# Codes4Fun/moshi.cpp

Measured on AMD Instinct MI355X. Metric: audio frames/sec (12.5 Hz target) moshika-7B q4_k decode, higher is better.
Workload: dtype q4_K weights x q8_K activations (int8 dot, f32 accumulate); bf16 KV; f32 elsewhere; 1 GPU; moshi-sts --bench loop: mimi encode + Temporal step + 8 Depth steps + mimi decode, moshika q4_k, 1 audio stream per GPU, greedy, ctx capacity 3000; context_fill_start=0, parallelism=1 GPU, device= (gfx950:sramecc+:xnack-)

## Files before the change

moshi.cpp_amd/csrc/hip_backend.hip:

```cpp
#include "hip_common.h"
#include "ggml-cpu.h"

#include <string.h>

#include <algorithm>
#include <functional>
#include <deque>
#include <map>
#include <memory>
#include <set>
#include <string>
#include <unordered_map>
#include <vector>

#define UPLOAD_SLOTS       8
#define UPLOAD_BLOB_BYTES  (64 * 1024)
#define UPLOAD_MAX_DESCS   1024
#define READBACK_PINNED_BYTES (64 * 1024)
#define AGET_SLOTS 64
#define AGET_SLOT_BYTES 256
#define UPLOAD_SMALL_MAX   16384

struct plan_t;

// ... 2516 lines not shown
            const ggml_tensor * n = g->nodes[i];
            const bool layout = is_layout_op(n->op);
            if (!layout || it != pl.at_pos.end())
                fprintf(stderr, "plan %4d %-18s [%5lld %5lld %4lld %2lld] %s%s%s\n", i, ggml_op_name(n->op), (long long) n->ne[0], (long long) n->ne[1], (long long) n->ne[2],
                        (long long) n->ne[3], pl.an.skip[(size_t) i] ? "fused" : (layout ? "-" : "GENERIC"), it != pl.at_pos.end() ? " <emit group>" : "", n->view_src ? " (alias)" : "");
        }
        if (!pl.an.skip[(size_t) i]) {
            if (g->nodes[i]->op == GGML_OP_SOFT_MAX || g->nodes[i]->op == GGML_OP_SET_ROWS) pl.p->n_generic_attn_nodes++;
            emit_generic(pl.em, g->nodes[i]);
        }
        if (it != pl.at_pos.end()) for (auto & f : it->second) pl.p->steps.push_back(f);
    }
}

static void hoist_rope_tables(planner & pl) {
    plan_t * p = pl.p;
    for (size_t i = 1; i + 1 < p->steps.size(); i++) {
        pstep & h = p->steps[i];
        const pstep & m = p->steps[i - 1];
        if (!h.hoist_dst || !m.is_mv || m.mv.special || m.mv.wtype != GGML_TYPE_F32 || m.mv.ncols != 2 || !p->steps[i + 1].is_mv) continue;
        auto clash = [&](const float * q, int64_t n_floats) { return q && (const char *) q < h.hoist_dst + h.hoist_bytes && h.hoist_dst < (const char *) (q + n_floats); };
        const mv_args & a = m.mv;
        if (clash(a.x, a.x_cs * (a.ncols - 1) + a.K) || clash(a.y, a.y_cs * (a.ncols - 1) + a.M) || clash(a.x_out, a.K * a.ncols) || clash(a.residual, a.r_cs * (a.ncols - 1) + a.M) ||
            clash(a.alpha, a.K) || clash(a.beta, a.K)) continue;
        std::swap(p->steps[i - 1], p->steps[i]);
    }
}

static bool chains_wanted(const planner & pl) {
    return pl.fuse && pl.keep && !(pl.c->flags & 16) && ((pl.c->flags & 32) || k_chain_default_on()) && spin_kernels_possible(pl.c);
// ... 377 lines not shown
```

moshi.cpp_amd/csrc/hip_chain.hip:

```cpp
#include "hip_common.h"
#include "hip_device.h"
#include "hip_mv_device.h"
#include "hip_attn_body.h"

#include <stdlib.h>
#include <string.h>
#include <type_traits>
#include <map>
#include <vector>

#define CH_NCW       8
#define CH_THREADS   (CH_NCW * 64)
#define CH_PMAX_OF(G) ((G) >= 256 ? 2 : (G) >= 128 ? 3 : 6)
#define CH_XF_MAX    4096
#define CH_PART_MAX  2048
#define CH_RES_MAX   256
#define CH_ATTW      1408
#define CH_SPIN_MAX  (1u << 24)
#define CH_MAX_PHASES 4095

typedef unsigned long long u64;

#if defined(CH_LOG)
__device__ u64 g_ch_log[2][512][16];
// ... 1135 lines not shown
        if (!mimi_is_mv(op, D, D, MV_PLAIN) || op.x != at.out || op.x_cs != D || op.residual != xin || op.r_cs != xin_cs || op.out_act) { if (verbose && d.L == 0) fprintf(stderr, "mimi_match: rule %d fails at layer 0\n", 8); break; }
        if (!mimi_is_mv(l1, D, F, MV_LAYERNORM) || !l1.alpha || l1.x != op.y || l1.x_cs != D || l1.residual || l1.out_scale || l1.out_act != 1) { if (verbose && d.L == 0) fprintf(stderr, "mimi_match: rule %d fails at layer 0\n", 9); break; }
        if (!mimi_is_mv(l2, F, D, MV_PLAIN) || l2.x != l1.y || l2.x_cs != F || l2.residual != op.y || l2.r_cs != D || l2.out_act) { if (verbose && d.L == 0) fprintf(stderr, "mimi_match: rule %d fails at layer 0\n", 10); break; }
        if (d.L == 0 && d.x_cs < D) { if (verbose && d.L == 0) fprintf(stderr, "mimi_match: rule %d fails at layer 0\n", 11); break; }
        d.mv.push_back({ ip.w, ip.alpha, ip.beta, nullptr, ip.y, ip.x_out, ip.eps, { 0, 0, 0 } });
        d.mv.push_back({ op.w, nullptr, nullptr, op.out_scale, op.y, nullptr, 0.f, { 0, 0, 0 } });
        d.mv.push_back({ l1.w, l1.alpha, l1.beta, nullptr, l1.y, l1.x_out, l1.eps, { 0, 0, 0 } });
        d.mv.push_back({ l2.w, nullptr, nullptr, l2.out_scale, l2.y, nullptr, 0.f, { 0, 0, 0 } });
        d.at.push_back({ at.kcache, at.vcache, at.rot, at.mask, at.index, at.out });
        d.weight_bytes += ip.M * ip.row_bytes + op.M * op.row_bytes + l1.M * l1.row_bytes + l2.M * l2.row_bytes;
        xprev = l2.y; xprev_cs = D;
        d.L++;
        i += 5;
    }
    if (d.L < 2) return 0;
    d.len = i;
    return i;
}
static size_t mimi_attn_smem(const attn_args & at) { return ATTN_RING256_SMEM + (size_t) at.C * 4 + (size_t) at.T * at.D * 4 * 3 + (size_t) CH_NCW * 64 * 8 * 8 + 16 + (size_t) at.T * at.C * 4 + 64; }
static size_t mimi_smem_bytes(const mimi_desc & d) {
    return (size_t) (2 * MIMI_F + 8) * 4 + 16 * 8 + sizeof(chain_ctl) + ((mimi_attn_smem(d.at0) + 15) & ~(size_t) 15) + d.mv.size() * sizeof(mimi_mv) + d.at.size() * sizeof(mimi_at);
}
static size_t mimi_tables_bytes(const mimi_desc & d) { return GGML_PAD(d.mv.size() * sizeof(mimi_mv) + d.at.size() * sizeof(mimi_at), 256); }
static bool mimi_resident(const mimi_desc & d, int usable_cus) {
    const size_t smem = mimi_smem_bytes(d);
    if (smem > 159 * 1024) return false;
    static bool granted = false;
    if (!granted) { HIP_CHECK(hipFuncSetAttribute((const void *) mimi_tr_kernel, hipFuncAttributeMaxDynamicSharedMemorySize, 159 * 1024)); granted = true; }
    static const int force = chain_env("MI355X_CHAIN_GRID_FORCE", 0);
    int per_cu = 0;
    return force || (hipOccupancyMaxActiveBlocksPerMultiprocessor(&per_cu, (const void *) mimi_tr_kernel, CH_THREADS, smem) == hipSuccess && (long long) per_cu * usable_cus >= 256);
}

struct smp_strip { std::vector<mv_args> mv; std::vector<const sample_args *> smp; std::vector<int> end_of; bool any = false; };
static unsigned g_sampled_ticket;
static void sampled_strip(const mv_args * mv, int n, smp_strip & o) {
    for (int i = 0; i < n; i++) {
        const mv_args & a = mv[i];
        if (!a.special) { o.mv.push_back(a); o.smp.push_back(nullptr); o.end_of.push_back(i + 1); continue; }
        if (a.special != 3 || o.mv.empty() || o.smp.back() || !a.smp) break;
        mv_args & hd = o.mv.back();
        const sample_args & sa = *a.smp;
        if (hd.ticket || hd.argmax_out[0] || hd.argmax_out[1] || sa.logits != hd.y || sa.n != hd.M || sa.n != 2048 || sa.k < 1 || sa.k > 256 || !sa.noise || !sa.out) break;
        hd.ticket = &g_sampled_ticket; hd.argmax_out[0] = sa.out; hd.argmax_out[1] = sa.out2;
        o.smp.back() = a.smp; o.end_of.back() = i + 1; o.any = true;
    }
// ... 214 lines not shown
            char * state = base + mimi_tables_bytes(d);
            std::vector<char> tab(mimi_tables_bytes(d), 0);
            memcpy(tab.data(), d.mv.data(), d.mv.size() * sizeof(mimi_mv));
            memcpy(tab.data() + d.mv.size() * sizeof(mimi_mv), d.at.data(), d.at.size() * sizeof(mimi_at));
            c->nest_tables.swap(tab);
            HIP_CHECK(hipMemcpyAsync(base, c->nest_tables.data(), c->nest_tables.size(), hipMemcpyHostToDevice, s));
            HIP_CHECK(hipMemsetAsync(state, 0, chain_state_bytes(256), s));
            mimi_params & N = c->MM;
            memset(&N, 0, sizeof(N));
            N.P.phases = nullptr; N.P.n_phases = d.len;
            N.P.launch_seq = (unsigned *) state; N.P.gbuf = (u64 *) (state + 256); N.P.cand = N.P.gbuf + 2 * CH_XF_MAX; N.P.err = err; N.P.delay = 0;
            N.tables = (const u32x4 *) base;
            N.n_layers = d.L; N.x_in = d.x_in; N.x_cs = d.x_cs;
            N.at = d.at0; N.at.q = N.at.k = N.at.v = nullptr;
            N.first_partial = d.first_partial ? 1 : 0;
            if (d.first_partial) { N.q0 = d.at_first.q; N.k0 = d.at_first.k; N.v0 = d.at_first.v; }
            N.q_off = d.q_off; N.k_off = d.k_off; N.v_off = d.v_off;
            N.attn_smem = mimi_attn_smem(d.at0);
            N.ring256 = chain_env("MI355X_ATTN_RING256", 1) && d.at0.C > 64 && d.at0.C <= 256 ? 1 : 0;
            {
                static const int dflt[2] = { 30, 200 };
                N.delay[0] = dflt[0]; N.delay[1] = dflt[1];
                if (const char * e = getenv("MI355X_MIMI_DELAY")) { int v[2]; const int got = sscanf(e, "%d,%d", &v[0], &v[1]); for (int i = 0; i < got && i < 2; i++) N.delay[i] = v[i] < 0 ? 0 : v[i] > 600 ? 600 : v[i]; }
            }
            c->P = N.P;
            c->smem = mimi_smem_bytes(d);
            c->mimi = true; c->n80_weight_bytes = d.weight_bytes; c->n80_len = d.len;
            if (chain_env("MI355X_CHAIN_VERBOSE", 0)) fprintf(stderr, "chain engine: Mimi transformer program, %d layers, ring of %d, %zu bytes of LDS, %d plan steps\n", d.L, d.at0.C, c->smem, d.len);
            return c;
        }
    }
    {
        n80_desc d;
        if (n > 0 && (mv[0].special == 2 || (!mv[0].special && mv[0].wtype == GGML_TYPE_Q8_0)) && c->grid == 256 && nest80_match(mv, n, d) == n) {
            char * base = (char *) ws;
            char * state = base + nest80_tables_bytes(d);
            char * din = state + chain_state_bytes(256);
            std::vector<char> tab(nest80_tables_bytes(d), 0);
            char * t = tab.data();
            memcpy(t, d.ph.data(), d.ph.size() * sizeof(nest_ph)); t += d.ph.size() * sizeof(nest_ph);
            memcpy(t, d.at.data(), d.at.size() * sizeof(n80_at)); t += d.at.size() * sizeof(n80_at);
            memcpy(t, d.st.data(), d.st.size() * sizeof(n80_st)); t += d.st.size() * sizeof(n80_st);
            memcpy(t, d.dsets.data(), d.dsets.size() * 8);
// ... 72 lines not shown
    for (size_t i = 0; i < c->phases.size(); i++) {
        chain_phase & ph = c->phases[i];
        if (ph.attn >= 0) ph.at = c->attns[(size_t) ai++];
        ph.n_in = i > 0 ? c->phases[i - 1].n_pub : 0;
        ph.kind = chain_shape_kind(ph, c->grid);
        if (ph.emb_chain) { ph.prev_out[0] = c->phases[i - 1].argmax_out[0]; ph.prev_out[1] = c->phases[i - 1].argmax_out[1]; }
    }
}
void k_chain_free(chain_plan * c) { delete c; }
int k_chain_length(const chain_plan * c) { return c->P.n_phases; }
int64_t k_chain_weight_bytes(const chain_plan * c) { if (c->nest80 || c->mimi) return c->n80_weight_bytes; int64_t b = 0; for (auto & ph : c->phases) b += (int64_t) ph.M * ph.row_bytes; return b; }

bool k_chain_is_step_program(const chain_plan * c) { return c->nest || c->nest80 || c->mimi; }

void k_chain_launch(hipStream_t s, const chain_plan * c) {
    if (c->mimi) { mimi_tr_kernel<<<256, CH_THREADS, c->smem, s>>>(c->MM); return; }
    if (c->nest80) { depth_nest80_kernel<2048, 2048><<<256, CH_THREADS, c->smem, s>>>(c->N80); return; }
    if (c->nest) {
        if (c->NP.head_argmax == 2) depth_nest_kernel<256, true><<<c->grid, CH_THREADS, c->nest_smem, s>>>(c->NP);
        else depth_nest_kernel<256><<<c->grid, CH_THREADS, c->nest_smem, s>>>(c->NP);
        return;
    }
    if (c->grid == 256) matvec_chain_kernel<256><<<c->grid, CH_THREADS, c->smem, s>>>(c->P);
    else if (c->grid == 128) matvec_chain_kernel<128><<<c->grid, CH_THREADS, c->smem, s>>>(c->P);
    else matvec_chain_kernel<64><<<c->grid, CH_THREADS, c->smem, s>>>(c->P);
}

#define VQC_CPW 4
#define VQC_LEVELS_MAX 32
struct vqc_level { const char * emb; long long emb_row_bytes; const float * add_c; const float * num; float * resid_out; float * idx_f; int32_t * idx_i; long long pad; };
static_assert(sizeof(vqc_level) == 64, "level records are read by 16-byte lanes");
// ... 133 lines not shown
```

moshi.cpp_amd/csrc/hip_chain_mimi.h:

```cpp
#pragma once

struct mimi_mv { const char * w; const float * alpha; const float * beta; const float * out_scale; float * y; float * x_out; float eps; int pad[3]; };
struct mimi_at { char * kcache; char * vcache; const float * rot; const float * mask; const int32_t * index; float * out; };
static_assert(sizeof(mimi_mv) == 64 && sizeof(mimi_at) == 48, "tables are copied to LDS by 16-byte lanes");

struct mimi_params {
    chain_params P;
    const u32x4 * tables;
    int n_layers;
    const float * x_in; int64_t x_cs;
    attn_args at;
    int q_off, k_off, v_off;
    size_t attn_smem;
    int ring256;
    int first_partial;
    const float * q0, * k0, * v0;
    int delay[2];
};
#define MIMI_D 512
#define MIMI_F 2048

__global__ void __launch_bounds__(CH_THREADS) mimi_tr_kernel(mimi_params N) {
    constexpr int G = 256, D = MIMI_D, F = MIMI_F, T = 2;
    extern __shared__ __attribute__((aligned(16))) char smem[];
    const int tid = threadIdx.x, lane = tid & 63;
    const int wave = __builtin_amdgcn_readfirstlane(tid >> 6);
    const int wg = blockIdx.x;
    const int L = N.n_layers;

    float * xs = (float *) smem;
    float * xres = xs + T * F;
    double * stat = (double *) (xres + 8);
    chain_ctl * ctl = (chain_ctl *) (stat + 16);
    char * at_smem = (char *) (ctl + 1);
    const mimi_mv * t_mv = (const mimi_mv *) (at_smem + ((N.attn_smem + 15) & ~(size_t) 15));
    const mimi_at * t_at = (const mimi_at *) (t_mv + 4 * L);

    const chain_params & P = N.P;
    auto nbar = [&]() { lds_barrier(); };
    if (tid == 0) { ctl->failed = 0; ctl->token = 0; }
    {
        const int n16 = (4 * L * (int) sizeof(mimi_mv) + L * (int) sizeof(mimi_at)) / 16;
        const GLOBAL_AS u32x4 * src = (const GLOBAL_AS u32x4 *) N.tables;
        for (int i = tid; i < n16; i += CH_THREADS) ((u32x4 *) t_mv)[i] = src[i];
    }
    const unsigned launch = *gp(P.launch_seq);
    const unsigned tag_base = launch << 12;
    __syncthreads();

    auto ld_mv = [&](int q) {
        mimi_mv r;
        unsigned w[16];
        const unsigned * s = (const unsigned *) (t_mv + q);
#pragma unroll
        for (int i = 0; i < 16; i++) w[i] = (unsigned) __builtin_amdgcn_readfirstlane((int) s[i]);
        __builtin_memcpy(&r, w, sizeof(r));
        return r;
    };
    auto ld_w = [&](int q) -> const char * {
        const unsigned * s = (const unsigned *) (t_mv + q);
        unsigned w[2] = { (unsigned) __builtin_amdgcn_readfirstlane((int) s[0]), (unsigned) __builtin_amdgcn_readfirstlane((int) s[1]) };
        const char * r;
        __builtin_memcpy(&r, w, 8);
        return r;
    };
    auto ld_at = [&](int q) {
        mimi_at r;
        unsigned w[12];
        const unsigned * s = (const unsigned *) (t_at + q);
#pragma unroll
        for (int i = 0; i < 12; i++) w[i] = (unsigned) __builtin_amdgcn_readfirstlane((int) s[i]);
        __builtin_memcpy(&r, w, sizeof(r));
        return r;
    };
    auto give_up = [&]() { if (lane == 0) { lds_store(&ctl->failed, 1u); *gp(P.err) = 2u; } };

    f32x4 wr[8];
    auto request = [&](auto kvc, const char * w, int rows) {
        constexpr int KV = decltype(kvc)::value;
        const int row = wg * rows + (wave < rows ? wave : rows - 1);
        const GLOBAL_AS char * src = gp(w) + (long long) row * (KV * 256 * 4);
#pragma unroll
        for (int it = 0; it < KV; it++) wr[it] = __builtin_nontemporal_load((const GLOBAL_AS f32x4 *) (src + ((long long) it * 256 + lane * 4) * 4));
    };
    if (N.first_partial) request(std::integral_constant<int, 2>(), ld_w(1), 2); else request(std::integral_constant<int, 2>(), ld_w(0), 6);

    const int col = wave >> 2, t256 = (wave & 3) * 64 + lane;
    auto poll_cols = [&](auto kvc, int p, float xr[], int delay) {
        constexpr int KV = decltype(kvc)::value;
        for (int i = 0; i < delay; i++) __builtin_amdgcn_s_sleep(1);
        const unsigned tag_in = tag_base | (unsigned) p;
        const u64 * gin = P.gbuf + (size_t) ((p - 1) & 1) * CH_XF_MAX + (size_t) col * (KV * 256) + t256;
        u64 g[KV];
        unsigned spins = 0;
        for (;;) {
#pragma unroll
            for (int j = 0; j < KV; j++) g[j] = __hip_atomic_load(gin + 256 * j, __ATOMIC_RELAXED, __HIP_MEMORY_SCOPE_AGENT);
            bool ok = true;
#pragma unroll
            for (int j = 0; j < KV; j++) ok = ok && (unsigned) (g[j] >> 32) == tag_in;
            if (__all(ok)) break;
            if (++spins > CH_SPIN_MAX || lds_load(&ctl->failed)) { give_up(); break; }
            __builtin_amdgcn_s_sleep(1);
        }
        settle_vmcnt();
#pragma unroll
        for (int j = 0; j < KV; j++) xr[j] = __uint_as_float((unsigned) g[j]);
    };
    auto col_sum = [&](double v, int slot) -> double {
        v = wave_allsum_f64(v);
        if (lane == 0) stat[slot * 8 + wave] = v;
        nbar();
        const double * s4 = stat + slot * 8 + col * 4;
        return s4[0] + s4[1] + s4[2] + s4[3];
    };
    auto layer_norm = [&](float xr[2], const mimi_mv & mv) {
        const float al[2] = { gp(mv.alpha)[t256], gp(mv.alpha)[t256 + 256] };
        float be[2] = { 0.f, 0.f };
        if (mv.beta) { be[0] = gp(mv.beta)[t256]; be[1] = gp(mv.beta)[t256 + 256]; }
        double acc = 0;
#pragma unroll
        for (int j = 0; j < 2; j++) acc += (double) xr[j];
        acc = col_sum(acc, 0);
        const float mean = (float) (acc / (double) D);
        acc = 0;
#pragma unroll
        for (int j = 0; j < 2; j++) { const float v = xr[j] - mean; acc += (double) (v * v); }
        acc = col_sum(acc, 1);
        const float scale = 1.0f / sqrtf((float) (acc / (double) D) + mv.eps);
#pragma unroll
        for (int j = 0; j < 2; j++) { float v = ((xr[j] - mean) * scale) * al[j]; if (mv.beta) v = v + be[j]; xr[j] = v; }
    };
    auto row_dot = [&](auto kvc, float out[2]) {
        constexpr int KV = decltype(kvc)::value, K = KV * 256;
        double acc[2] = { 0, 0 };
#pragma unroll
        for (int it = 0; it < KV; it++) {
            const int k = it * 256 + lane * 4;
#pragma unroll
            for (int c = 0; c < 2; c++) {
                const float4 xv = *(const float4 *) (xs + c * K + k);
                acc[c] += (double) (wr[it][0] * xv.x);
                acc[c] += (double) (wr[it][1] * xv.y);
                acc[c] += (double) (wr[it][2] * xv.z);
                acc[c] += (double) (wr[it][3] * xv.w);
            }
// ... 2 lines not shown
        for (int c = 0; c < 2; c++) out[c] = (float) wave_allsum_f64(acc[c]);
    };
    auto publish = [&](int p, int M, int row, const float v[2]) {
        const unsigned tag_out = tag_base | (unsigned) (p + 1);
        u64 * go = P.gbuf + (size_t) (p & 1) * CH_XF_MAX;
#pragma unroll
        for (int c = 0; c < 2; c++) st_granule(go + (size_t) c * M + row, tag_out, __float_as_uint(v[c]));
    };
    [[maybe_unused]] constexpr int grid = G;
    const int owner_idx = wg >> 4;
    const bool owner = (wg & 15) == (owner_idx & 7);

    int p = 0;
#pragma unroll 1
    for (int l = 0; l < L; l++) {
        if (l == 0 && N.first_partial) {
            if (wave < 2) {
#pragma unroll
                for (int c = 0; c < 2; c++) if (lane == c) xres[c * 2 + wave] = gp(N.x_in)[(int64_t) c * N.x_cs + wg * 2 + wave];
            }
            p = __builtin_amdgcn_readfirstlane(p + 1);
        } else {
            CH_STAMP(10);
            const mimi_mv mv = ld_mv(4 * l);
            float xr[2];
            if (l == 0) { xr[0] = gp(N.x_in)[(int64_t) col * N.x_cs + t256]; xr[1] = gp(N.x_in)[(int64_t) col * N.x_cs + t256 + 256]; }
            else poll_cols(std::integral_constant<int, 2>(), p, xr, N.delay[0]);
            if (l == 0 && wave < 2) {
#pragma unroll
                for (int c = 0; c < 2; c++) if (lane == c) xres[c * 2 + wave] = gp(N.x_in)[(int64_t) c * N.x_cs + wg * 2 + wave];
            }
            CH_STAMP(2);
            layer_norm(xr, mv);
            xs[col * D + t256] = xr[0]; xs[col * D + t256 + 256] = xr[1];
            if (mv.x_out && wg == 0) { gp(mv.x_out)[(int64_t) col * D + t256] = xr[0]; gp(mv.x_out)[(int64_t) col * D + t256 + 256] = xr[1]; }
            nbar();
            CH_STAMP(5);
            if (wave < 6) {
                float o[2];
                row_dot(std::integral_constant<int, 2>(), o);
                const int row = wg * 6 + wave;
                if (lane == 0) { publish(p, 3 * D, row, o); gp(mv.y)[row] = o[0]; gp(mv.y)[3 * D + row] = o[1]; }
            }
            request(std::integral_constant<int, 2>(), ld_w(4 * l + 1), 2);
            CH_STAMP(8);
            p = __builtin_amdgcn_readfirstlane(p + 1);
        }
        {
            CH_STAMP(10);
            if (owner) {
                const mimi_at ta = ld_at(l);
                attn_args at = N.at;
                at.kcache = ta.kcache; at.vcache = ta.vcache; at.rot = ta.rot; at.mask = ta.mask; at.index = ta.index; at.out = ta.out;
                at.q = nullptr; at.k = nullptr; at.v = nullptr;
                at.row_split = 1; at.n_groups = 0; at.write_only = 0;
                const attn_split_ws w0 = { nullptr, nullptr, nullptr, 1, P.err, 0, 1 << 30, 1 << 30 };
                const attn_gqkv gq = { P.gbuf + (size_t) ((p - 1) & 1) * CH_XF_MAX, (int64_t) N.q_off, (int64_t) N.k_off, (int64_t) N.v_off, P.err };
                attn_gout go = { P.gbuf + (size_t) (p & 1) * CH_XF_MAX, tag_base | (unsigned) (p + 1), (int64_t) D };
#if defined(CH_LOG)
                go.log = wg == 0 && p < 512 ? &g_ch_log[0][p][0] : nullptr;
#endif
                __syncthreads();
                if (l == 0 && N.first_partial) {
                    at.q = N.q0; at.k = N.k0; at.v = N.v0;
                    if (N.ring256) attn_ring256_body<AT_GOUT>(at, at_smem, owner_idx >> 1, owner_idx & 1, 0u, attn_gqkv(), go);
                    else attn_decode_body<false, CH_NCW, AT_GOUT>(at, w0, at_smem, owner_idx >> 1, 0, owner_idx & 1, 0u, attn_gqkv(), go);
                } else if (N.ring256) attn_ring256_body<AT_GQKV | AT_GOUT>(at, at_smem, owner_idx >> 1, owner_idx & 1, tag_base | (unsigned) p, gq, go);
                else attn_decode_body<false, CH_NCW, AT_GQKV | AT_GOUT>(at, w0, at_smem, owner_idx >> 1, 0, owner_idx & 1, tag_base | (unsigned) p, gq, go);
                __syncthreads();
                CH_STAMP(8);
            }
            p = __builtin_amdgcn_readfirstlane(p + 1);
        }
        {
            CH_STAMP(10);
            const mimi_mv mv = ld_mv(4 * l + 1);
            float osc = 1.f;
            if (mv.out_scale && wave < 2) osc = gp(mv.out_scale)[wg * 2 + wave];
            float xr[2];
            poll_cols(std::integral_constant<int, 2>(), p, xr, owner ? 0 : N.delay[1]);
            CH_STAMP(2);
            xs[col * D + t256] = xr[0]; xs[col * D + t256 + 256] = xr[1];
            nbar();
            CH_STAMP(5);
            if (wave < 2) {
                float o[2];
                row_dot(std::integral_constant<int, 2>(), o);
                const int row = wg * 2 + wave;
                if (lane == 0) {
#pragma unroll
                    for (int c = 0; c < 2; c++) { float s = o[c]; if (mv.out_scale) s = s * osc; s = xres[c * 2 + wave] + s; o[c] = s; xres[c * 2 + wave] = s; }
                    publish(p, D, row, o); gp(mv.y)[row] = o[0]; gp(mv.y)[D + row] = o[1];
                }
            }
            request(std::integral_constant<int, 2>(), ld_w(4 * l + 2), 8);
            CH_STAMP(8);
            p = __builtin_amdgcn_readfirstlane(p + 1);
        }
        {
            CH_STAMP(10);
            const mimi_mv mv = ld_mv(4 * l + 2);
            float xr[2];
            poll_cols(std::integral_constant<int, 2>(), p, xr, N.delay[0]);
            CH_STAMP(2);
            layer_norm(xr, mv);
            xs[col * D + t256] = xr[0]; xs[col * D + t256 + 256] = xr[1];
            if (mv.x_out && wg == 0) { gp(mv.x_out)[(int64_t) col * D + t256] = xr[0]; gp(mv.x_out)[(int64_t) col * D + t256 + 256] = xr[1]; }
            nbar();
            {
                float o[2];
                row_dot(std::integral_constant<int, 2>(), o);
                const int row = wg * 8 + wave;
                if (lane == 0) { o[0] = gelu_table(o[0]); o[1] = gelu_table(o[1]); publish(p, F, row, o); gp(mv.y)[row] = o[0]; gp(mv.y)[F + row] = o[1]; }
            }
            request(std::integral_constant<int, 8>(), ld_w(4 * l + 3), 2);
            CH_STAMP(8);
            p = __builtin_amdgcn_readfirstlane(p + 1);
        }
        {
            CH_STAMP(10);
            const mimi_mv mv = ld_mv(4 * l + 3);
            float osc = 1.f;
            if (mv.out_scale && wave < 2) osc = gp(mv.out_scale)[wg * 2 + wave];
            float xr[8];
            poll_cols(std::integral_constant<int, 8>(), p, xr, N.delay[0]);
            CH_STAMP(2);
#pragma unroll
            for (int j = 0; j < 8; j++) xs[col * F + t256 + 256 * j] = xr[j];
            nbar();
            if (wave < 2) {
                float o[2];
                row_dot(std::integral_constant<int, 8>(), o);
                const int row = wg * 2 + wave;
                if (lane == 0) {
#pragma unroll
                    for (int c = 0; c < 2; c++) { float s = o[c]; if (mv.out_scale) s = s * osc; s = xres[c * 2 + wave] + s; o[c] = s; xres[c * 2 + wave] = s; }
                    if (l + 1 < L) publish(p, D, row, o);
                    gp(mv.y)[row] = o[0]; gp(mv.y)[D + row] = o[1];
                }
            }
            if (l + 1 < L) request(std::integral_constant<int, 2>(), ld_w(4 * l + 4), 6);
            nbar();
            CH_STAMP(8);
            p = __builtin_amdgcn_readfirstlane(p + 1);
        }
    }
    if (wg == 0 && tid == 0) *gp(P.launch_seq) = launch + 1u;
}
```

moshi.cpp_amd/csrc/moshi_hot.cpp:

```cpp
#include "moshi_hot.h"
#include "delay_ring.h"
#include "gguf.h"
#include "ggml-cpu.h"

#include <dlfcn.h>
#include <math.h>
#include <stdlib.h>
#include <string.h>

#include <deque>
#include <functional>
#include <map>
#include <set>
#include <string>
#include <vector>

typedef struct ggml_tensor * T;

namespace {

struct Rng {
    uint64_t s;
    explicit Rng(uint64_t seed) : s(seed) {}
    uint64_t next() { uint64_t z = (s += 0x9E3779B97F4A7C15ull); z = (z ^ (z >> 30)) * 0xBF58476D1CE4E5B9ull; z = (z ^ (z >> 27)) * 0x94D049BB133111EBull; return z ^ (z >> 31); }
// ... 734 lines not shown
    int (*rccl_all_reduce)(const void *, void *, size_t, int, int, void *, void *) = nullptr;
    moshi_hot_allreduce_t tp_allreduce = nullptr; void * tp_allreduce_user = nullptr;
    int64_t tp_reductions = 0;
    Transformer temporal_tp; T tp_x = nullptr, tp_msg = nullptr; std::vector<Builder *> g_tp;
    bool tp_frame = false; T tp_in = nullptr; Builder * g_tp_pre = nullptr, * g_tp_import = nullptr, * g_tp_post = nullptr; int64_t tp_frames = 0;
    DelayProtocol proto; DelayRing ring;
    struct Column { DelayRing ring; int64_t pos = 0; bool open = false, held = false; };
    int n_streams = 1; ModelKind kind = ModelKind::single; std::vector<Column> cols;
    struct Sampling { moshi_hot_sampling s; bool seeded = false; };
    std::vector<Sampling> sampling; bool any_seeded = false, sampling_dirty = true;
    T inv_temp_text = nullptr, inv_temp = nullptr;

    Rvq rvq_first, rvq_rest;
    ConvTr upsample; Conv downsample;
    Transformer dec_tr, enc_tr;
    std::vector<Conv> dec_convs; std::vector<ConvTr> dec_convtrs; std::vector<ResBlock> dec_res;
    std::vector<Conv> enc_convs; std::vector<ResBlock> enc_res;
    Builder * g_dec = nullptr; T dec_codes = nullptr, dec_frame = nullptr; int dec_T = 0;
    Builder * g_enc = nullptr; T enc_frame = nullptr, enc_codes = nullptr; int enc_T = 0;
    T enc_latent[2] = { nullptr, nullptr };

    std::vector<int32_t> tokens_tmp;
    std::vector<int32_t> pipe_codes, pipe_tokens; bool pipe_have_codes = false, pipe_have_tokens = false; float pipe_vad = 0.f;
    bool temporal_staged = false;
    std::function<void()> after_temporal_launch;
    int32_t last_text = 0; std::vector<int32_t> last_audio;
    bool timing = false; double phase_us[4] = { 0, 0, 0, 0 }; int64_t phase_n[4] = { 0, 0, 0, 0 };
};

#define STREAMS_REFUSE(ret) do { if (m->n_streams > 1) return ret; } while (0)

namespace {

T state(moshi_hot_model * m, enum ggml_type type, int64_t n0, int64_t n1 = 1, int64_t n2 = 1) {
    T t = ggml_new_tensor_3d(m->st_ctx, type, n0, n1, n2);
    return t;
}
T state4(moshi_hot_model * m, enum ggml_type type, int64_t n0, int64_t n1, int64_t n2, int64_t n3) {
    T t = ggml_new_tensor_4d(m->st_ctx, type, n0, n1, n2, n3);
    return t;
}

bool owns_step(const moshi_hot_config & c, int k) { return c.dep_shard_world <= 1 || k % c.dep_shard_world == c.dep_shard_rank; }

void make_transformer(moshi_hot_model * m, Transformer & tr, const std::string & name, int dim, int heads, int n_layers, int ffn_hidden,
                      int capacity, int max_period, int n_weight_sets, bool mimi_style, enum ggml_type wtype, int cross_len = 0, bool norms_only = false) {
    Weights & W = *m->W;
    tr.dim = dim; tr.heads = heads; tr.capacity = capacity; tr.max_period = max_period;
    tr.layers.resize((size_t) n_layers);
    const float s_in = 1.f / sqrtf((float) dim);
    const float upd = m->cfg.update_scale > 0.f ? m->cfg.update_scale : 1.f;
    auto qgen = [](float sd) { return [sd](T t, Rng & r, std::vector<uint8_t> & o) { gen_quant(t, r, o, sd); }; };
    auto ones = [](T t, Rng &, std::vector<uint8_t> & o) { gen_const(t, 1.f, o); };
    auto zeros = [](T t, Rng &, std::vector<uint8_t> & o) { gen_const(t, 0.f, o); };
    for (int l = 0; l < n_layers; l++) {
        Layer & L = tr.layers[(size_t) l];
        const std::string p = name + ".layers." + std::to_string(l) + ".";
        if (mimi_style) {
// ... 218 lines not shown
    m->g_dec = new Builder(m->be_codec, 256);
    Builder & g = *m->g_dec;
    T codes = ggml_new_tensor_2d(g, GGML_TYPE_I32, 1, c.mimi_n_q);
    m->dec_codes = codes;
    const int64_t B = codes->ne[2], K = codes->ne[1], Tn = codes->ne[0];
    T first = ggml_view_3d(g, codes, Tn, 1, B, codes->nb[1], codes->nb[2], 0);
    T emb = rvq_decode(g, m->rvq_first, first);
    if (K > 1) {
        T rest = ggml_view_3d(g, codes, Tn, K - 1, B, codes->nb[1], codes->nb[2], codes->nb[1] * 1);
        emb = ggml_add(g, emb, rvq_decode(g, m->rvq_rest, rest));
    }
    emb = streaming_conv_transpose(g, m->upsample, emb);
    m->dec_T = (int) emb->ne[0];
    T x = ggml_cont(g, ggml_transpose(g, emb));
    x = transformer_graph_build(g, m->dec_tr, x);
    x = ggml_transpose(g, x);
    x = streaming_conv(g, m->dec_convs[0], x);
    x = ggml_elu(g, x);
    for (int i = 0; i < 4; i++) {
        x = streaming_conv_transpose(g, m->dec_convtrs[(size_t) i], x);
        x = resnet_block(g, m->dec_res[(size_t) i], x);
        x = ggml_elu(g, x);
    }
    x = streaming_conv(g, m->dec_convs[1], x);
    m->dec_frame = x;
    g.expand(x);
    g.alloc();
}

void build_encode_graph(moshi_hot_model * m) {
// ... 1 lines not shown
    m->g_enc = new Builder(m->be_codec, 256);
    Builder & g = *m->g_enc;
    T x = ggml_new_tensor_1d(g, GGML_TYPE_F32, 1920);
    m->enc_frame = x;
    x = streaming_conv(g, m->enc_convs[0], x);
    for (int i = 0; i < 4; i++) {
        x = resnet_block(g, m->enc_res[(size_t) i], x);
        x = ggml_elu(g, x);
        x = streaming_conv(g, m->enc_convs[(size_t) (1 + i)], x);
    }
    x = ggml_elu(g, x);
    x = streaming_conv(g, m->enc_convs[5], x);
    m->enc_T = (int) x->ne[0];
    x = ggml_cont(g, ggml_transpose(g, x));
    x = transformer_graph_build(g, m->enc_tr, x);
    x = ggml_transpose(g, x);
    x = streaming_conv(g, m->downsample, x);
    T codes = rvq_encode(g, m->rvq_first, x, &m->enc_latent[0]);
    if (c.mimi_n_q > 1) codes = ggml_concat(g, codes, rvq_encode(g, m->rvq_rest, x, &m->enc_latent[1]), 1);
    codes = ggml_cast(g, codes, GGML_TYPE_I32);
    m->enc_codes = codes;
    g.expand(codes);
    g.alloc();
}

}

extern "C" void moshi_hot_config_moshika(struct moshi_hot_config * c) {
    memset(c, 0, sizeof(*c));
    c->dim = 4096; c->num_heads = 32; c->num_layers = 32; c->ffn_hidden = 11264; c->context = 3000; c->max_period = 10000;
// ... 265 lines not shown
        p.delays.assign(c.delays, c.delays + p.cols());
        for (int d : p.delays) if (d > p.max_delay) p.max_delay = d;
        p.rows = p.max_delay + 2 + (c.personaplex ? 1 : 0);
        p.initial.assign((size_t) p.cols(), c.card); p.initial[0] = c.text_card;
        DelayRing fresh; fresh.p = &p; fresh.reset();
        if (m->n_streams > 1) m->cols.assign((size_t) m->n_streams, { fresh, 0, kind == ModelKind::lockstep }); else m->ring = fresh;
    }
    if (c.enable_mimi_decoder || c.enable_mimi_encoder) {
        W.part = c.enable_mimi_decoder ? 3 : 2;
        make_rvq(m, m->rvq_first, "mimi.quantizer.rvq_first", 1, c.mimi_codebook_size);
        make_rvq(m, m->rvq_rest, "mimi.quantizer.rvq_rest", c.mimi_n_q > 1 ? c.mimi_n_q - 1 : 0, c.mimi_codebook_size);
    }
    if (c.enable_mimi_decoder) {
        W.part = 3;
        m->upsample = make_convtr(m, "mimi.upsample.convtr", 512, 512, 4, 2, 512, false, 1);
        make_transformer(m, m->dec_tr, "mimi.decoder_transformer.transformer", 512, 8, 8, 2048, 250, 10000, 1, true, GGML_TYPE_F32);
        m->dec_convs.push_back(make_conv(m, "mimi.decoder.model.0.conv", 512, 1024, 7, 1, true, true));
        const int ch[5] = { 1024, 512, 256, 128, 64 }, ks[4] = { 16, 12, 10, 8 }, st[4] = { 8, 6, 5, 4 };
        int64_t len = 2;
        for (int i = 0; i < 4; i++) {
            m->dec_convtrs.push_back(make_convtr(m, "mimi.decoder.model." + std::to_string(2 + 3 * i) + ".convtr", ch[i], ch[i + 1], ks[i], st[i], 1, true, len));
            len = len * st[i];
            m->dec_res.push_back(make_res(m, "mimi.decoder.model." + std::to_string(3 + 3 * i), ch[i + 1]));
        }
        m->dec_convs.push_back(make_conv(m, "mimi.decoder.model.14.conv", 64, 1, 3, 1, true, true));
    }
    if (c.enable_mimi_encoder) {
        W.part = 2;
        m->enc_convs.push_back(make_conv(m, "mimi.encoder.model.0.conv", 1, 64, 7, 1, true, true));
        const int ch[5] = { 64, 128, 256, 512, 1024 }, ks[4] = { 8, 10, 12, 16 }, st[4] = { 4, 5, 6, 8 };
        for (int i = 0; i < 4; i++) {
            m->enc_res.push_back(make_res(m, "mimi.encoder.model." + std::to_string(1 + 3 * i), ch[i]));
            m->enc_convs.push_back(make_conv(m, "mimi.encoder.model." + std::to_string(3 + 3 * i) + ".conv", ch[i], ch[i + 1], ks[i], st[i], true, true));
        }
        m->enc_convs.push_back(make_conv(m, "mimi.encoder.model.14.conv", 1024, 512, 3, 1, true, true));
        make_transformer(m, m->enc_tr, "mimi.encoder_transformer.transformer", 512, 8, 8, 2048, 250, 10000, 1, true, GGML_TYPE_F32);
        m->downsample = make_conv(m, "mimi.downsample.conv", 512, 512, 4, 2, false, true);
    }
    W.load();
    m->st_buf = ggml_backend_alloc_ctx_tensors(m->st_ctx, backend);
    if (!m->st_buf && m->n_streams > 1) {
        moshi_hot_free(m);
        return nullptr;
    }
    GGML_ASSERT(m->st_buf);
    ggml_backend_buffer_clear(m->st_buf, 0);
    m->tokens_tmp.resize((size_t) (c.n_q + 1 + 32));
    m->pipe_codes.resize((size_t) (c.n_q + 1 + 32)); m->pipe_tokens.resize((size_t) (c.n_q + 1 + 32));
    ggml_backend_synchronize(backend);
    return m;
}
// ... 1399 lines not shown
}

extern "C" float moshi_hot_sts_pipeline_vad(moshi_hot_model_t * m) { return m->pipe_vad; }
extern "C" int64_t moshi_hot_offset(moshi_hot_model_t * m) { return m->kind == ModelKind::lockstep ? m->cols[0].ring.frames : m->ring.frames; }
extern "C" void moshi_hot_last_raw_tokens(moshi_hot_model_t * m, int32_t * text_token, int32_t * audio_tokens) {
    *text_token = m->last_text;
    for (size_t i = 0; i < m->last_audio.size(); i++) audio_tokens[i] = m->last_audio[i];
}
extern "C" size_t moshi_hot_weight_bytes(moshi_hot_model_t * m, int part) { return part >= 0 && part < 6 ? m->W->bytes[part] : 0; }
extern "C" int moshi_hot_read_last(moshi_hot_model_t * m, const char * what, float * out, int64_t n) {
    T t = nullptr;
    if (!strcmp(what, "text_logits")) t = m->text_logits;
    else if (!strcmp(what, "transformer_out")) t = m->transformer_out;
    else if (!strcmp(what, "transformer_in")) t = m->g_transformer_in;
    else if (!strcmp(what, "stack_out")) t = m->g_stack_out;
    else if (!strcmp(what, "enc_latent_first")) t = m->enc_latent[0];
    else if (!strcmp(what, "enc_latent_rest")) t = m->enc_latent[1];
    else if (!strncmp(what, "dep_logits", 10)) { const int k = atoi(what + 10); if (k >= 0 && k < (int) m->dep_logits.size()) t = m->dep_logits[(size_t) k]; }
    if (!t || ggml_nelements(t) < n) return -1;
    ggml_backend_tensor_get(t, out, 0, (size_t) n * 4);
    return 0;
}
extern "C" struct ggml_cgraph * moshi_hot_graph(moshi_hot_model_t * m, int which) {
    Builder * b = which == 0 ? m->g_temporal : which == 1 ? m->g_depth : which == 2 ? m->g_enc : which == 3 ? m->g_dec : nullptr;
    return b ? b->gf : nullptr;
}
extern "C" struct ggml_tensor * moshi_hot_weight(moshi_hot_model_t * m, const char * name) {
    auto it = m->W->by_name.find(name);
    return it == m->W->by_name.end() ? nullptr : it->second;
}
extern "C" void moshi_hot_set_timing(moshi_hot_model_t * m, int on) { m->timing = on != 0; for (int i = 0; i < 4; i++) { m->phase_us[i] = 0; m->phase_n[i] = 0; } }
extern "C" void moshi_hot_get_timing(moshi_hot_model_t * m, double * us_per_call) { for (int i = 0; i < 4; i++) us_per_call[i] = m->phase_n[i] ? m->phase_us[i] / (double) m->phase_n[i] : 0.0; }
extern "C" void moshi_hot_force_last(moshi_hot_model_t * m, int32_t text_token, const int32_t * audio_tokens) { STREAMS_REFUSE();
    m->ring.force_last(text_token, audio_tokens);
    m->tok_state_for = -1;
}
extern "C" void moshi_hot_set_context_fill(moshi_hot_model_t * m, int64_t offset) {
    if (m->kind == ModelKind::slots) return;
    if (m->kind == ModelKind::lockstep) { for (auto & col : m->cols) col.pos = offset; return; }
    unstage_temporal(m);
    m->temporal.offset = (int) offset;
    if (m->tp_x) m->temporal_tp.offset = (int) offset;
}

extern "C" int64_t moshi_hot_ring_bytes(moshi_hot_model_t * m, int which, int layer, int kv, void * buf, int64_t nbytes, int write) { STREAMS_REFUSE(-1);
    Transformer & tr = which == 0 ? m->temporal : m->depth;
    if (layer < 0 || layer >= (int) tr.layers.size()) return -1;
    T t = kv == 0 ? tr.layers[(size_t) layer].kcache : tr.layers[(size_t) layer].vcache;
    if (!t) return -1;
    const int64_t size = (int64_t) ggml_nbytes(t);
    if (buf) {
        const size_t n = (size_t) (nbytes < size ? nbytes : size);
        if (write) ggml_backend_tensor_set(t, buf, 0, n); else ggml_backend_tensor_get(t, buf, 0, n);
    }
    return size;
}

extern "C" void moshi_hot_fill_ring(moshi_hot_model_t * m, int which, int layer, uint64_t seed, float scale) { STREAMS_REFUSE();
    Transformer & tr = which == 0 ? m->temporal : m->depth;
    for (int l = 0; l < (int) tr.layers.size(); l++) {
        if (layer >= 0 && l != layer) continue;
// ... 45 lines not shown
```

Before: 459.4 frames/s.

## Template Mimi transformer kernel on ring256 and first-partial, load descriptor fields lazily

The Mimi codec transformer kernel becomes a template on whether ring-256 attention is used and whether the first layer starts mid-layer, so the unused attention body is compiled out. Per-step descriptor loads switch from a full 16-word readfirstlane copy to loading only the fields each phase needs, which is meant to cut SGPR pressure and scalar loads. The first-partial path now republishes the precomputed QKV output instead of running attention from separate pointers, with a matching host-side check. Debug hooks are added as well: env switches for ring capacity and rope hoisting, and readback of encoder and decoder transformer outputs.

```diff
diff --git a/moshi.cpp_amd/csrc/hip_backend.hip b/moshi.cpp_amd/csrc/hip_backend.hip
--- a/moshi.cpp_amd/csrc/hip_backend.hip
+++ b/moshi.cpp_amd/csrc/hip_backend.hip
@@ -2554,6 +2554,7 @@
 }
 
 static void hoist_rope_tables(planner & pl) {
+    if (const char * e = getenv("MI355X_HOIST_ROPE")) if (atoi(e) == 0) return;
     plan_t * p = pl.p;
     for (size_t i = 1; i + 1 < p->steps.size(); i++) {
         pstep & h = p->steps[i];
diff --git a/moshi.cpp_amd/csrc/hip_chain.hip b/moshi.cpp_amd/csrc/hip_chain.hip
--- a/moshi.cpp_amd/csrc/hip_chain.hip
+++ b/moshi.cpp_amd/csrc/hip_chain.hip
@@ -1173,6 +1173,11 @@
         i += 5;
     }
     if (d.L < 2) return 0;
+    if (d.first_partial) {
+        const attn_args & f = d.at_first, & o = d.at0;
+        if (f.q - d.q_off != f.k - d.k_off || f.q - d.q_off != f.v - d.v_off || f.C != o.C || f.scale != o.scale || f.k_nb1 != o.k_nb1 || f.k_nb2 != o.k_nb2 ||
+            f.v_nb1 != o.v_nb1 || f.v_nb2 != o.v_nb2 || (f.rot != nullptr) != (o.rot != nullptr)) return 0;
+    }
     d.len = i;
     return i;
 }
@@ -1181,14 +1186,22 @@
     return (size_t) (2 * MIMI_F + 8) * 4 + 16 * 8 + sizeof(chain_ctl) + ((mimi_attn_smem(d.at0) + 15) & ~(size_t) 15) + d.mv.size() * sizeof(mimi_mv) + d.at.size() * sizeof(mimi_at);
 }
 static size_t mimi_tables_bytes(const mimi_desc & d) { return GGML_PAD(d.mv.size() * sizeof(mimi_mv) + d.at.size() * sizeof(mimi_at), 256); }
+static bool mimi_ring256(const mimi_desc & d) { return chain_env("MI355X_ATTN_RING256", 1) && d.at0.C > 64 && d.at0.C <= 256; }
+typedef void (*mimi_kernel_t)(mimi_params);
+static mimi_kernel_t mimi_kernel_for(bool ring256, bool first_partial) {
+    return ring256 ? (first_partial ? mimi_tr_kernel<true, true> : mimi_tr_kernel<true, false>) : (first_partial ? mimi_tr_kernel<false, true> : mimi_tr_kernel<false, false>);
+}
 static bool mimi_resident(const mimi_desc & d, int usable_cus) {
     const size_t smem = mimi_smem_bytes(d);
     if (smem > 159 * 1024) return false;
-    static bool granted = false;
-    if (!granted) { HIP_CHECK(hipFuncSetAttribute((const void *) mimi_tr_kernel, hipFuncAttributeMaxDynamicSharedMemorySize, 159 * 1024)); granted = true; }
+    const bool ring256 = mimi_ring256(d);
+    const void * fn = (const void *) mimi_kernel_for(ring256, d.first_partial);
+    static bool granted[4] = { false, false, false, false };
+    bool & g = granted[(ring256 ? 2 : 0) + (d.first_partial ? 1 : 0)];
+    if (!g) { HIP_CHECK(hipFuncSetAttribute(fn, hipFuncAttributeMaxDynamicSharedMemorySize, 159 * 1024)); g = true; }
     static const int force = chain_env("MI355X_CHAIN_GRID_FORCE", 0);
     int per_cu = 0;
-    return force || (hipOccupancyMaxActiveBlocksPerMultiprocessor(&per_cu, (const void *) mimi_tr_kernel, CH_THREADS, smem) == hipSuccess && (long long) per_cu * usable_cus >= 256);
+    return force || (hipOccupancyMaxActiveBlocksPerMultiprocessor(&per_cu, fn, CH_THREADS, smem) == hipSuccess && (long long) per_cu * usable_cus >= 256);
 }
 
 struct smp_strip { std::vector<mv_args> mv; std::vector<const sample_args *> smp; std::vector<int> end_of; bool any = false; };
@@ -1433,10 +1446,10 @@
             N.n_layers = d.L; N.x_in = d.x_in; N.x_cs = d.x_cs;
             N.at = d.at0; N.at.q = N.at.k = N.at.v = nullptr;
             N.first_partial = d.first_partial ? 1 : 0;
-            if (d.first_partial) { N.q0 = d.at_first.q; N.k0 = d.at_first.k; N.v0 = d.at_first.v; }
+            if (d.first_partial) N.y0 = d.at_first.q - d.q_off;
             N.q_off = d.q_off; N.k_off = d.k_off; N.v_off = d.v_off;
             N.attn_smem = mimi_attn_smem(d.at0);
-            N.ring256 = chain_env("MI355X_ATTN_RING256", 1) && d.at0.C > 64 && d.at0.C <= 256 ? 1 : 0;
+            N.ring256 = mimi_ring256(d) ? 1 : 0;
             {
                 static const int dflt[2] = { 30, 200 };
                 N.delay[0] = dflt[0]; N.delay[1] = dflt[1];
@@ -1445,7 +1458,7 @@
             c->P = N.P;
             c->smem = mimi_smem_bytes(d);
             c->mimi = true; c->n80_weight_bytes = d.weight_bytes; c->n80_len = d.len;
-            if (chain_env("MI355X_CHAIN_VERBOSE", 0)) fprintf(stderr, "chain engine: Mimi transformer program, %d layers, ring of %d, %zu bytes of LDS, %d plan steps\n", d.L, d.at0.C, c->smem, d.len);
+            if (chain_env("MI355X_CHAIN_VERBOSE", 0)) fprintf(stderr, "chain engine: Mimi transformer program, %d layers, ring of %d, %zu bytes of LDS, %d plan steps, %s attention body, first layer %s\n", d.L, d.at0.C, c->smem, d.len, N.ring256 ? "ring-256" : "general", N.first_partial ? "from its attention" : "whole");
             return c;
         }
     }
@@ -1548,7 +1561,7 @@
 bool k_chain_is_step_program(const chain_plan * c) { return c->nest || c->nest80 || c->mimi; }
 
 void k_chain_launch(hipStream_t s, const chain_plan * c) {
-    if (c->mimi) { mimi_tr_kernel<<<256, CH_THREADS, c->smem, s>>>(c->MM); return; }
+    if (c->mimi) { mimi_kernel_for(c->MM.ring256 != 0, c->MM.first_partial != 0)<<<256, CH_THREADS, c->smem, s>>>(c->MM); return; }
     if (c->nest80) { depth_nest80_kernel<2048, 2048><<<256, CH_THREADS, c->smem, s>>>(c->N80); return; }
     if (c->nest) {
         if (c->NP.head_argmax == 2) depth_nest_kernel<256, true><<<c->grid, CH_THREADS, c->nest_smem, s>>>(c->NP);
diff --git a/moshi.cpp_amd/csrc/hip_chain_mimi.h b/moshi.cpp_amd/csrc/hip_chain_mimi.h
--- a/moshi.cpp_amd/csrc/hip_chain_mimi.h
+++ b/moshi.cpp_amd/csrc/hip_chain_mimi.h
@@ -14,12 +14,13 @@
     size_t attn_smem;
     int ring256;
     int first_partial;
-    const float * q0, * k0, * v0;
+    const float * y0;
     int delay[2];
 };
 #define MIMI_D 512
 #define MIMI_F 2048
 
+template <bool RING256, bool FIRST_PARTIAL>
 __global__ void __launch_bounds__(CH_THREADS) mimi_tr_kernel(mimi_params N) {
     constexpr int G = 256, D = MIMI_D, F = MIMI_F, T = 2;
     extern __shared__ __attribute__((aligned(16))) char smem[];
@@ -48,22 +49,16 @@
     const unsigned tag_base = launch << 12;
     __syncthreads();
 
-    auto ld_mv = [&](int q) {
-        mimi_mv r;
-        unsigned w[16];
-        const unsigned * s = (const unsigned *) (t_mv + q);
-#pragma unroll
-        for (int i = 0; i < 16; i++) w[i] = (unsigned) __builtin_amdgcn_readfirstlane((int) s[i]);
-        __builtin_memcpy(&r, w, sizeof(r));
-        return r;
-    };
-    auto ld_w = [&](int q) -> const char * {
-        const unsigned * s = (const unsigned *) (t_mv + q);
+    auto ld_ptr = [&](const void * field) -> const char * {
+        const unsigned * s = (const unsigned *) field;
         unsigned w[2] = { (unsigned) __builtin_amdgcn_readfirstlane((int) s[0]), (unsigned) __builtin_amdgcn_readfirstlane((int) s[1]) };
         const char * r;
         __builtin_memcpy(&r, w, 8);
         return r;
     };
+    auto ld_w = [&](int q) -> const char * { return ld_ptr(&t_mv[q].w); };
+    auto ld_y = [&](int q) -> float * { return (float *) ld_ptr(&t_mv[q].y); };
+    auto ld_eps = [&](int q) -> float { return __int_as_float(__builtin_amdgcn_readfirstlane(__float_as_int(t_mv[q].eps))); };
     auto ld_at = [&](int q) {
         mimi_at r;
         unsigned w[12];
@@ -83,7 +78,7 @@
 #pragma unroll
         for (int it = 0; it < KV; it++) wr[it] = __builtin_nontemporal_load((const GLOBAL_AS f32x4 *) (src + ((long long) it * 256 + lane * 4) * 4));
     };
-    if (N.first_partial) request(std::integral_constant<int, 2>(), ld_w(1), 2); else request(std::integral_constant<int, 2>(), ld_w(0), 6);
+    if (FIRST_PARTIAL) request(std::integral_constant<int, 2>(), ld_w(1), 2); else request(std::integral_constant<int, 2>(), ld_w(0), 6);
 
     const int col = wave >> 2, t256 = (wave & 3) * 64 + lane;
     auto poll_cols = [&](auto kvc, int p, float xr[], int delay) {
@@ -114,10 +109,14 @@
         const double * s4 = stat + slot * 8 + col * 4;
         return s4[0] + s4[1] + s4[2] + s4[3];
     };
-    auto layer_norm = [&](float xr[2], const mimi_mv & mv) {
-        const float al[2] = { gp(mv.alpha)[t256], gp(mv.alpha)[t256 + 256] };
-        float be[2] = { 0.f, 0.f };
-        if (mv.beta) { be[0] = gp(mv.beta)[t256]; be[1] = gp(mv.beta)[t256 + 256]; }
+    auto ln_load = [&](int q, float al[2], float be[2]) -> bool {
+        const float * alpha = (const float *) ld_ptr(&t_mv[q].alpha), * beta = (const float *) ld_ptr(&t_mv[q].beta);
+        al[0] = gp(alpha)[t256]; al[1] = gp(alpha)[t256 + 256];
+        be[0] = be[1] = 0.f;
+        if (beta) { be[0] = gp(beta)[t256]; be[1] = gp(beta)[t256 + 256]; }
+        return beta != nullptr;
+    };
+    auto layer_norm = [&](float xr[2], const float al[2], const float be[2], const bool has_beta, const float eps) {
         double acc = 0;
 #pragma unroll
         for (int j = 0; j < 2; j++) acc += (double) xr[j];
@@ -127,9 +126,9 @@
 #pragma unroll
         for (int j = 0; j < 2; j++) { const float v = xr[j] - mean; acc += (double) (v * v); }
         acc = col_sum(acc, 1);
-        const float scale = 1.0f / sqrtf((float) (acc / (double) D) + mv.eps);
-#pragma unroll
-        for (int j = 0; j < 2; j++) { float v = ((xr[j] - mean) * scale) * al[j]; if (mv.beta) v = v + be[j]; xr[j] = v; }
+        const float scale = 1.0f / sqrtf((float) (acc / (double) D) + eps);
+#pragma unroll
+        for (int j = 0; j < 2; j++) { float v = ((xr[j] - mean) * scale) * al[j]; if (has_beta) v = v + be[j]; xr[j] = v; }
     };
     auto row_dot = [&](auto kvc, float out[2]) {
         constexpr int KV = decltype(kvc)::value, K = KV * 256;
@@ -162,15 +161,21 @@
     int p = 0;
 #pragma unroll 1
     for (int l = 0; l < L; l++) {
-        if (l == 0 && N.first_partial) {
+        if (FIRST_PARTIAL && l == 0) {
             if (wave < 2) {
 #pragma unroll
                 for (int c = 0; c < 2; c++) if (lane == c) xres[c * 2 + wave] = gp(N.x_in)[(int64_t) c * N.x_cs + wg * 2 + wave];
             }
+            if (wave < 6 && lane == 0) {
+                const int row = wg * 6 + wave;
+                const float o[2] = { gp(N.y0)[row], gp(N.y0)[3 * D + row] };
+                publish(p, 3 * D, row, o);
+            }
             p = __builtin_amdgcn_readfirstlane(p + 1);
         } else {
             CH_STAMP(10);
-            const mimi_mv mv = ld_mv(4 * l);
+            float al[2], be[2];
+            const bool has_beta = ln_load(4 * l, al, be);
             float xr[2];
             if (l == 0) { xr[0] = gp(N.x_in)[(int64_t) col * N.x_cs + t256]; xr[1] = gp(N.x_in)[(int64_t) col * N.x_cs + t256 + 256]; }
             else poll_cols(std::integral_constant<int, 2>(), p, xr, N.delay[0]);
@@ -179,16 +184,16 @@
                 for (int c = 0; c < 2; c++) if (lane == c) xres[c * 2 + wave] = gp(N.x_in)[(int64_t) c * N.x_cs + wg * 2 + wave];
             }
             CH_STAMP(2);
-            layer_norm(xr, mv);
+            layer_norm(xr, al, be, has_beta, ld_eps(4 * l));
             xs[col * D + t256] = xr[0]; xs[col * D + t256 + 256] = xr[1];
-            if (mv.x_out && wg == 0) { gp(mv.x_out)[(int64_t) col * D + t256] = xr[0]; gp(mv.x_out)[(int64_t) col * D + t256 + 256] = xr[1]; }
+            if (wg == 0) { float * x_out = (float *) ld_ptr(&t_mv[4 * l].x_out); if (x_out) { gp(x_out)[(int64_t) col * D + t256] = xr[0]; gp(x_out)[(int64_t) col * D + t256 + 256] = xr[1]; } }
             nbar();
             CH_STAMP(5);
             if (wave < 6) {
                 float o[2];
                 row_dot(std::integral_constant<int, 2>(), o);
                 const int row = wg * 6 + wave;
-                if (lane == 0) { publish(p, 3 * D, row, o); gp(mv.y)[row] = o[0]; gp(mv.y)[3 * D + row] = o[1]; }
+                if (lane == 0) { float * y = ld_y(4 * l); publish(p, 3 * D, row, o); gp(y)[row] = o[0]; gp(y)[3 * D + row] = o[1]; }
             }
             request(std::integral_constant<int, 2>(), ld_w(4 * l + 1), 2);
             CH_STAMP(8);
@@ -202,19 +207,17 @@
                 at.kcache = ta.kcache; at.vcache = ta.vcache; at.rot = ta.rot; at.mask = ta.mask; at.index = ta.index; at.out = ta.out;
                 at.q = nullptr; at.k = nullptr; at.v = nullptr;
                 at.row_split = 1; at.n_groups = 0; at.write_only = 0;
-                const attn_split_ws w0 = { nullptr, nullptr, nullptr, 1, P.err, 0, 1 << 30, 1 << 30 };
                 const attn_gqkv gq = { P.gbuf + (size_t) ((p - 1) & 1) * CH_XF_MAX, (int64_t) N.q_off, (int64_t) N.k_off, (int64_t) N.v_off, P.err };
                 attn_gout go = { P.gbuf + (size_t) (p & 1) * CH_XF_MAX, tag_base | (unsigned) (p + 1), (int64_t) D };
 #if defined(CH_LOG)
                 go.log = wg == 0 && p < 512 ? &g_ch_log[0][p][0] : nullptr;
 #endif
                 __syncthreads();
-                if (l == 0 && N.first_partial) {
-                    at.q = N.q0; at.k = N.k0; at.v = N.v0;
-                    if (N.ring256) attn_ring256_body<AT_GOUT>(at, at_smem, owner_idx >> 1, owner_idx & 1, 0u, attn_gqkv(), go);
-                    else attn_decode_body<false, CH_NCW, AT_GOUT>(at, w0, at_smem, owner_idx >> 1, 0, owner_idx & 1, 0u, attn_gqkv(), go);
-                } else if (N.ring256) attn_ring256_body<AT_GQKV | AT_GOUT>(at, at_smem, owner_idx >> 1, owner_idx & 1, tag_base | (unsigned) p, gq, go);
-                else attn_decode_body<false, CH_NCW, AT_GQKV | AT_GOUT>(at, w0, at_smem, owner_idx >> 1, 0, owner_idx & 1, tag_base | (unsigned) p, gq, go);
+                if constexpr (RING256) attn_ring256_body<AT_GQKV | AT_GOUT>(at, at_smem, owner_idx >> 1, owner_idx & 1, tag_base | (unsigned) p, gq, go);
+                else {
+                    const attn_split_ws w0 = { nullptr, nullptr, nullptr, 1, P.err, 0, 1 << 30, 1 << 30 };
+                    attn_decode_body<false, CH_NCW, AT_GQKV | AT_GOUT>(at, w0, at_smem, owner_idx >> 1, 0, owner_idx & 1, tag_base | (unsigned) p, gq, go);
+                }
                 __syncthreads();
                 CH_STAMP(8);
             }
@@ -222,9 +225,9 @@
         }
         {
             CH_STAMP(10);
-            const mimi_mv mv = ld_mv(4 * l + 1);
+            const float * out_scale = (const float *) ld_ptr(&t_mv[4 * l + 1].out_scale);
             float osc = 1.f;
-            if (mv.out_scale && wave < 2) osc = gp(mv.out_scale)[wg * 2 + wave];
+            if (out_scale && wave < 2) osc = gp(out_scale)[wg * 2 + wave];
             float xr[2];
             poll_cols(std::integral_constant<int, 2>(), p, xr, owner ? 0 : N.delay[1]);
             CH_STAMP(2);
@@ -237,8 +240,9 @@
                 const int row = wg * 2 + wave;
                 if (lane == 0) {
 #pragma unroll
-                    for (int c = 0; c < 2; c++) { float s = o[c]; if (mv.out_scale) s = s * osc; s = xres[c * 2 + wave] + s; o[c] = s; xres[c * 2 + wave] = s; }
-                    publish(p, D, row, o); gp(mv.y)[row] = o[0]; gp(mv.y)[D + row] = o[1];
+                    for (int c = 0; c < 2; c++) { float s = o[c]; if (out_scale) s = s * osc; s = xres[c * 2 + wave] + s; o[c] = s; xres[c * 2 + wave] = s; }
+                    float * y = ld_y(4 * l + 1);
+                    publish(p, D, row, o); gp(y)[row] = o[0]; gp(y)[D + row] = o[1];
                 }
             }
             request(std::integral_constant<int, 2>(), ld_w(4 * l + 2), 8);
@@ -247,19 +251,20 @@
         }
         {
             CH_STAMP(10);
-            const mimi_mv mv = ld_mv(4 * l + 2);
+            float al[2], be[2];
+            const bool has_beta = ln_load(4 * l + 2, al, be);
             float xr[2];
             poll_cols(std::integral_constant<int, 2>(), p, xr, N.delay[0]);
             CH_STAMP(2);
-            layer_norm(xr, mv);
+            layer_norm(xr, al, be, has_beta, ld_eps(4 * l + 2));
             xs[col * D + t256] = xr[0]; xs[col * D + t256 + 256] = xr[1];
-            if (mv.x_out && wg == 0) { gp(mv.x_out)[(int64_t) col * D + t256] = xr[0]; gp(mv.x_out)[(int64_t) col * D + t256 + 256] = xr[1]; }
+            if (wg == 0) { float * x_out = (float *) ld_ptr(&t_mv[4 * l + 2].x_out); if (x_out) { gp(x_out)[(int64_t) col * D + t256] = xr[0]; gp(x_out)[(int64_t) col * D + t256 + 256] = xr[1]; } }
             nbar();
             {
                 float o[2];
                 row_dot(std::integral_constant<int, 2>(), o);
                 const int row = wg * 8 + wave;
-                if (lane == 0) { o[0] = gelu_table(o[0]); o[1] = gelu_table(o[1]); publish(p, F, row, o); gp(mv.y)[row] = o[0]; gp(mv.y)[F + row] = o[1]; }
+                if (lane == 0) { float * y = ld_y(4 * l + 2); o[0] = gelu_table(o[0]); o[1] = gelu_table(o[1]); publish(p, F, row, o); gp(y)[row] = o[0]; gp(y)[F + row] = o[1]; }
             }
             request(std::integral_constant<int, 8>(), ld_w(4 * l + 3), 2);
             CH_STAMP(8);
@@ -267,9 +272,9 @@
         }
         {
             CH_STAMP(10);
-            const mimi_mv mv = ld_mv(4 * l + 3);
+            const float * out_scale = (const float *) ld_ptr(&t_mv[4 * l + 3].out_scale);
             float osc = 1.f;
-            if (mv.out_scale && wave < 2) osc = gp(mv.out_scale)[wg * 2 + wave];
+            if (out_scale && wave < 2) osc = gp(out_scale)[wg * 2 + wave];
             float xr[8];
             poll_cols(std::integral_constant<int, 8>(), p, xr, N.delay[0]);
             CH_STAMP(2);
@@ -282,9 +287,10 @@
                 const int row = wg * 2 + wave;
                 if (lane == 0) {
 #pragma unroll
-                    for (int c = 0; c < 2; c++) { float s = o[c]; if (mv.out_scale) s = s * osc; s = xres[c * 2 + wave] + s; o[c] = s; xres[c * 2 + wave] = s; }
+                    for (int c = 0; c < 2; c++) { float s = o[c]; if (out_scale) s = s * osc; s = xres[c * 2 + wave] + s; o[c] = s; xres[c * 2 + wave] = s; }
                     if (l + 1 < L) publish(p, D, row, o);
-                    gp(mv.y)[row] = o[0]; gp(mv.y)[D + row] = o[1];
+                    float * y = ld_y(4 * l + 3);
+                    gp(y)[row] = o[0]; gp(y)[D + row] = o[1];
                 }
             }
             if (l + 1 < L) request(std::integral_constant<int, 2>(), ld_w(4 * l + 4), 6);
diff --git a/moshi.cpp_amd/csrc/moshi_hot.cpp b/moshi.cpp_amd/csrc/moshi_hot.cpp
--- a/moshi.cpp_amd/csrc/moshi_hot.cpp
+++ b/moshi.cpp_amd/csrc/moshi_hot.cpp
@@ -772,6 +772,7 @@
     Rvq rvq_first, rvq_rest;
     ConvTr upsample; Conv downsample;
     Transformer dec_tr, enc_tr;
+    T dec_tr_out = nullptr, enc_tr_out = nullptr;
     std::vector<Conv> dec_convs; std::vector<ConvTr> dec_convtrs; std::vector<ResBlock> dec_res;
     std::vector<Conv> enc_convs; std::vector<ResBlock> enc_res;
     Builder * g_dec = nullptr; T dec_codes = nullptr, dec_frame = nullptr; int dec_T = 0;
@@ -800,6 +801,12 @@
 }
 
 bool owns_step(const moshi_hot_config & c, int k) { return c.dep_shard_world <= 1 || k % c.dep_shard_world == c.dep_shard_rank; }
+
+int codec_ring_capacity() {
+    const char * e = getenv("MOSHI_HOT_MIMI_CONTEXT");
+    const int v = e ? atoi(e) : 0;
+    return v >= 2 && v <= 4096 ? v : 250;
+}
 
 void make_transformer(moshi_hot_model * m, Transformer & tr, const std::string & name, int dim, int heads, int n_layers, int ffn_hidden,
                       int capacity, int max_period, int n_weight_sets, bool mimi_style, enum ggml_type wtype, int cross_len = 0, bool norms_only = false) {
@@ -1048,6 +1055,7 @@
     m->dec_T = (int) emb->ne[0];
     T x = ggml_cont(g, ggml_transpose(g, emb));
     x = transformer_graph_build(g, m->dec_tr, x);
+    m->dec_tr_out = x;
     x = ggml_transpose(g, x);
     x = streaming_conv(g, m->dec_convs[0], x);
     x = ggml_elu(g, x);
@@ -1079,6 +1087,7 @@
     m->enc_T = (int) x->ne[0];
     x = ggml_cont(g, ggml_transpose(g, x));
     x = transformer_graph_build(g, m->enc_tr, x);
+    m->enc_tr_out = x;
     x = ggml_transpose(g, x);
     x = streaming_conv(g, m->downsample, x);
     T codes = rvq_encode(g, m->rvq_first, x, &m->enc_latent[0]);
@@ -1374,7 +1383,7 @@
     if (c.enable_mimi_decoder) {
         W.part = 3;
         m->upsample = make_convtr(m, "mimi.upsample.convtr", 512, 512, 4, 2, 512, false, 1);
-        make_transformer(m, m->dec_tr, "mimi.decoder_transformer.transformer", 512, 8, 8, 2048, 250, 10000, 1, true, GGML_TYPE_F32);
+        make_transformer(m, m->dec_tr, "mimi.decoder_transformer.transformer", 512, 8, 8, 2048, codec_ring_capacity(), 10000, 1, true, GGML_TYPE_F32);
         m->dec_convs.push_back(make_conv(m, "mimi.decoder.model.0.conv", 512, 1024, 7, 1, true, true));
         const int ch[5] = { 1024, 512, 256, 128, 64 }, ks[4] = { 16, 12, 10, 8 }, st[4] = { 8, 6, 5, 4 };
         int64_t len = 2;
@@ -1394,7 +1403,7 @@
             m->enc_convs.push_back(make_conv(m, "mimi.encoder.model." + std::to_string(3 + 3 * i) + ".conv", ch[i], ch[i + 1], ks[i], st[i], true, true));
         }
         m->enc_convs.push_back(make_conv(m, "mimi.encoder.model.14.conv", 1024, 512, 3, 1, true, true));
-        make_transformer(m, m->enc_tr, "mimi.encoder_transformer.transformer", 512, 8, 8, 2048, 250, 10000, 1, true, GGML_TYPE_F32);
+        make_transformer(m, m->enc_tr, "mimi.encoder_transformer.transformer", 512, 8, 8, 2048, codec_ring_capacity(), 10000, 1, true, GGML_TYPE_F32);
         m->downsample = make_conv(m, "mimi.downsample.conv", 512, 512, 4, 2, false, true);
     }
     W.load();
@@ -2824,6 +2833,8 @@
     else if (!strcmp(what, "transformer_out")) t = m->transformer_out;
     else if (!strcmp(what, "transformer_in")) t = m->g_transformer_in;
     else if (!strcmp(what, "stack_out")) t = m->g_stack_out;
+    else if (!strcmp(what, "enc_tr_out")) t = m->enc_tr_out;
+    else if (!strcmp(what, "dec_tr_out")) t = m->dec_tr_out;
     else if (!strcmp(what, "enc_latent_first")) t = m->enc_latent[0];
     else if (!strcmp(what, "enc_latent_rest")) t = m->enc_latent[1];
     else if (!strncmp(what, "dep_logits", 10)) { const int k = atoi(what + 10); if (k >= 0 && k < (int) m->dep_logits.size()) t = m->dep_logits[(size_t) k]; }
@@ -2854,7 +2865,7 @@
 }
 
 extern "C" int64_t moshi_hot_ring_bytes(moshi_hot_model_t * m, int which, int layer, int kv, void * buf, int64_t nbytes, int write) { STREAMS_REFUSE(-1);
-    Transformer & tr = which == 0 ? m->temporal : m->depth;
+    Transformer & tr = which == 0 ? m->temporal : which == 1 ? m->depth : which == 2 ? m->enc_tr : m->dec_tr;
     if (layer < 0 || layer >= (int) tr.layers.size()) return -1;
     T t = kv == 0 ? tr.layers[(size_t) layer].kcache : tr.layers[(size_t) layer].vcache;
     if (!t) return -1;
```

Measured after the change: 458.6 frames/s. Within noise of the previous version (-0.2%).
